# braingeneers/statdepth

Hardware: AMD Instinct MI355X
Metric: curve-pairs/sec (MBD) (higher is better)
Workload: dtype f64

## Files before the change

statdepth_amd/csrc/mbd_rank_bucket32.hip:

```cpp
#include <atomic>

#include "sd_common.h"
#include "rank_routes.h"
#include "rank_bucket.h"

namespace sd {

constexpr int R32_PRIO_LDS = 2;
constexpr int R32_PRIO_VALU = 0;
constexpr int R32_MIN_N = 3072;
constexpr int R32_LNB = 14;
constexpr int R32_NT = 512, R32_NW = 8;
constexpr int R32_LCAP = 64;
constexpr int R32_PAD = 12;
constexpr u32 R32_TB = 1024;
constexpr int R32_TSH = 30;
constexpr double R32_CDIV = 1.0 / 448.0;
constexpr double R32_BETA = 2.0;
constexpr double R32_VBASE = 274877906944.0;
constexpr u32 R32_VBASE_HI = 0x42500000u;
constexpr u32 R32_SENT = 0x7FFFFFFFu;

__device__ __forceinline__ u32 r32_word_offset(u32 vh) { return (vh << 2) & 0xFFFCu; }
__device__ __forceinline__ u32 r32_key_word(u32 off4, u32 par) { return (off4 << 5) | (par << 3); }
__device__ __forceinline__ u32 r32_key_word_offset(u32 kw) { return __builtin_amdgcn_ubfe(kw, 5u, 16u); }
__device__ __forceinline__ u32 r32_key_word_bucket(u32 kw) { return (__builtin_amdgcn_ubfe(kw, 7u, 14u) << 1) | ((kw >> 3) & 1u); }
__device__ __forceinline__ u32 r32_pair_word(u32 base, u32 h) { return __builtin_amdgcn_perm(base, h, 0x05040200u); }
__device__ __forceinline__ void r32_pair_decode(u32 pw, u32 kw, u32 &base, u32 &cnt) {
    cnt = __builtin_amdgcn_ubfe(pw, kw, 8u);
    base = (pw >> 16) + __builtin_amdgcn_ubfe(pw, 0u, kw);
}

template <int E, int LNB>
struct R32Cfg {
    static constexpr int NT = R32_NT, NW = R32_NW, NB = 1 << LNB;
    static constexpr int QW = NB / 2 / NT / 4;
    static_assert(QW >= 1 && NB / 2 == QW * 4 * NT, "whole quads of histogram words per thread");
    static constexpr int SH = 31 - LNB;
    static constexpr u32 C0 = R32_TB << SH, C1 = ((u32)NB - R32_TB) << SH;
    static constexpr u32 CU0 = 2u << SH, CU1 = ((u32)NB - 2u) << SH;
    static_assert(C0 % (2u << SH) == 0 && C1 % (2u << SH) == 0 && CU0 % (2u << SH) == 0 && CU1 % (2u << SH) == 0,
                  "the core's bounds are whole steps of the high word of 2^38 + image (2^18 images)");
    static constexpr u32 NANIMG = ((u32)NB + 2u) << SH;
    static_assert(LNB == 14, "the first tail octave continues the core's slope for 14 336 core buckets");
    static constexpr size_t HDR = 8 * NW * 8 + NW * 4 + 32 + (size_t)R32_LCAP * 8;
    static_assert(HDR % 16 == 0, "the histogram starts on a 16-byte boundary");
    static __host__ __device__ constexpr int al4(int n) { return (n + 3) & ~3; }
    static __host__ __device__ constexpr int pstride(int n) { return (n + 31) & ~31; }
    static __host__ __device__ constexpr int dummy_pos(int n) { return al4(n) + R32_PAD; }
    static __host__ __device__ constexpr size_t lds_bytes(int n) { return HDR + (size_t)(NB / 2 + 4) * 4 + (size_t)(dummy_pos(n) + 4) * 4; }
};

template <int E, int LNB>
__global__ __launch_bounds__(R32_NT, 4) void rank_bucket32_kernel(const double *__restrict__ Y, i64 n64, i64 row0, i64 rows,
                                                                 u32 *__restrict__ partial, unsigned char *__restrict__ rowflag,
                                                                 u32 *__restrict__ gate, u32 epoch, u64 *__restrict__ out_zero) {
    using C = R32Cfg<E, LNB>;
    constexpr int NT = C::NT, NW = C::NW, NB = C::NB, QW = C::QW, SH = C::SH;
    constexpr u32 C0 = C::C0, C1 = C::C1, CU0 = C::CU0, CU1 = C::CU1, NANIMG = C::NANIMG;
    constexpr size_t LDS = C::lds_bytes(E * NT);
    static_assert(2 * LDS <= 160 * 1024, "two workgroups per CU");
    static_assert(R32_PAD >= 0 && C::al4(E * NT) + 3 < C::dummy_pos(E * NT) + 4, "the second quad of the last bucket lies in S");
    __shared__ __attribute__((aligned(16))) double Sm[(LDS + 7) / 8];
    const int n = (int)n64;
    double *red = Sm;
    u32 *wtot = reinterpret_cast<u32 *>(red + 8 * NW);
    u32 *misc = wtot + NW;
    u32 *lkey = misc + 8, *lbe = lkey + R32_LCAP;
    u32 *H = reinterpret_cast<u32 *>(reinterpret_cast<char *>(Sm) + C::HDR);
    u32 *S = H + NB / 2 + 4;
    const unsigned short *H16 = reinterpret_cast<const unsigned short *>(H);
    const int t0 = threadIdx.x;
    const double INF = __builtin_huge_val();
    const double QNAN = __builtin_nan("");
    const int DUMMY = C::dummy_pos(n);
    const u32 nm1 = (u32)n - 1u;
    const u32 ranksum = (u32)(((u64)n * (u64)(n - 1)) >> 1);
    int t = t0;

    if (blockIdx.x == 0 && t == 0) gate[2] = 0;
    if (out_zero)
        for (i64 c = (i64)blockIdx.x * NT + t; c < n; c += (i64)gridDim.x * NT) out_zero[c] = 0;
    for (int p = n + t; p < DUMMY + 4; p += NT) S[p] = R32_SENT;
    {
        uint4 *Hq = reinterpret_cast<uint4 *>(H);
#pragma unroll
        for (int i = 0; i < QW; ++i) Hq[i * NT + t] = make_uint4(0, 0, 0, 0);
        if (t < 4) H[NB / 2 + t] = 0;
        if (t < 5) misc[t] = 0;
    }

    double x[E];
    auto load_row = [&](i64 r) {
        const double *rp = Y + (row0 + r) * n + t;
#pragma unroll
        for (int e = 0; e < E; ++e) x[e] = (e < E - 2 || t + e * NT < n) ? rp[e * NT] : QNAN;
    };
    u32 acc[E];
#pragma unroll
    for (int e = 0; e < E; ++e) acc[e] = 0;
    auto row_range = [&](int parity) {
        double mn = INF, mx = -INF;
#pragma unroll
        for (int e = 0; e < E; ++e) {
            mn = rb_mm<false>(mn, x[e]);
            mx = rb_mm<true>(mx, x[e]);
        }
        float2 wb = rb3_wave_bracket<E, NT>(mn, mx);
        {
            bool eqs = false;
#pragma unroll
            for (int e = 0; e < (E - 1 < 10 ? E - 1 : 10); ++e) eqs = eqs || (x[e] == x[e + 1]);
            if (__ballot(eqs) != 0) {
                float finf = __builtin_huge_valf();
                asm volatile("" : "+v"(finf));
                wb.x = finf;
                wb.y = -finf;
            }
        }
        const float imn = wb.x, imx = wb.y;
        mn = rb_wave_allreduce<false>(mn);
        mx = rb_wave_allreduce<true>(mx);
        double *rp = red + parity * 4 * NW;
        if ((t & 63) == 63) {
            double *wp = rp + 4 * (t >> 6);
            wp[0] = mn; wp[1] = mx;
            reinterpret_cast<float *>(wp + 2)[0] = imn;
            reinterpret_cast<float *>(wp + 2)[1] = imx;
        }
    };
    int par = 0;
    u32 rowidx = 0, nbad = 0, expect = 0;
    bool handover = false;
    bool stop = false;
    u32 kb[E];
    i64 r = blockIdx.x;
    for (; r < rows; r += gridDim.x) {
        t = t0;
        asm volatile("" : "+v"(t));
        const int lane = t & 63;
        const int wave = __builtin_amdgcn_readfirstlane(t >> 6);
        if (rowidx && t == 0) misc[3] = __hip_atomic_load(gate + 1, __ATOMIC_RELAXED, __HIP_MEMORY_SCOPE_AGENT);
        __builtin_amdgcn_s_setprio(R32_PRIO_LDS);
        load_row(r);
        row_range(par);
        double *redp = red + par * 4 * NW;
        par ^= 1;
        __syncthreads();
        if (rowidx) {
            const u32 w = misc[3];
            if ((w >> 8) == (epoch & 0xFFFFFFu) && (w & 0xFFu) >= 8u) { stop = true; break; }
        }
        double lo, hi;
        double mscale, moff, mc;
        u64 mcb;
        u32 mc0, mcw;
        u32 mh0, mhw;
        bool go, bad;
        {
            const double2 p = reinterpret_cast<const double2 *>(redp)[2 * (lane & (NW - 1))];
            const float2 pb = reinterpret_cast<const float2 *>(redp + 4 * (lane & (NW - 1)) + 2)[0];
            lo = rb_readlane_f64(rb_row_allreduce<false>(p.x), 0);
            hi = rb_readlane_f64(rb_row_allreduce<true>(p.y), 0);
            const double imn = (double)__int_as_float(__builtin_amdgcn_readfirstlane(__float_as_int(rb_row_allreduce_f32<true>(pb.x))));
            const double imx = (double)__int_as_float(__builtin_amdgcn_readfirstlane(__float_as_int(rb_row_allreduce_f32<false>(pb.y))));
            const bool fin = (hi > lo) && (lo > -INF) && (hi < INF) && ((hi - lo) < INF);
            bad = !fin && (hi >= lo);
            const double si = imx - imn;
            u32 c0 = CU0, c1 = CU1;
            if (fin && si > 0.0 && si < INF && (hi - lo) > (1.5 * (1.0 + 2.0 * R32_BETA)) * si) {
                const double lo2 = imn - R32_BETA * si, hi2 = imx + R32_BETA * si;
                lo = lo2 > lo ? lo2 : lo;
                hi = hi2 < hi ? hi2 : hi;
                c0 = C0;
                c1 = C1;
            }
            mc0 = c0;
            mcw = c1 - c0;
            const double wc = hi - lo;
            mscale = ((double)mcw - 64.0) / wc;
            moff = __builtin_fma(-lo, mscale, R32_VBASE + (double)c0);
            mh0 = R32_VBASE_HI + (c0 >> (SH + 1));
            mhw = mcw >> (SH + 1);
            mc = wc * R32_CDIV;
            mcb = (u64)__double_as_longlong(mc);
            go = fin && (wc > 0.0) && (mscale < INF) && (mc > 0.0);
            bad = bad || (fin && !go);
        }
        auto convert4 = [&](const double (&xv)[4], const bool (&isk)[4], u32 (&q)[4], u32 (&bk)[4]) {
            bool anyout = false;
            u32 vh[4];
#pragma unroll
            for (int i = 0; i < 4; ++i) {
                const u64 w = (u64)__double_as_longlong(__builtin_fma(xv[i], mscale, moff));
                vh[i] = (u32)(w >> 32);
                q[i] = (u32)w;
                anyout = anyout || (isk[i] && vh[i] - mh0 >= mhw);
            }
            if (__ballot(anyout) != 0) {
                const double vlo = __longlong_as_double((long long)((u64)mh0 << 32));
                double zero = 0.0;
                asm volatile("" : "+v"(zero));
#pragma unroll
                for (int i = 0; i < 4; ++i) {
                    const bool outc = vh[i] - mh0 >= mhw;
                    const bool low = __longlong_as_double((long long)(((u64)vh[i] << 32) | q[i])) < vlo;
                    double d = low ? lo - xv[i] : xv[i] - hi;
                    d = rb_mm<true>(d, zero);
                    const u64 tc = ((u64)__double_as_longlong(d + mc) - mcb) >> R32_TSH;
                    const u32 room = low ? mc0 - 1u : 0x7FFFFEFFu - (mc0 + mcw);
                    const u32 tcc = tc < (u64)room ? (u32)tc : room;
                    u32 qt = low ? (mc0 - 1u) - tcc : (mc0 + mcw) + tcc;
                    qt = (xv[i] == xv[i]) ? qt : NANIMG;
                    vh[i] = outc ? qt >> (SH + 1) : vh[i];
                    q[i] = outc ? qt << (31 - SH) : q[i];
                }
            }
#pragma unroll
            for (int i = 0; i < 4; ++i) {
                vh[i] = isk[i] ? vh[i] : NANIMG >> (SH + 1);
                q[i] = isk[i] ? q[i] : NANIMG << (31 - SH);
                bk[i] = vh[i];
            }
        };
        u32 bc[E];
        if (go) {

#pragma unroll
            for (int e0 = 0; e0 < E; e0 += 8) {
                u32 old[8];
#pragma unroll
                for (int h = 0; h < 8; h += 4) {
                    if (e0 + h < E) {
                        double xv[4];
                        u32 q[4], bk[4];
                        bool isk[4];
#pragma unroll
                        for (int i = 0; i < 4; ++i) {
                            const int e = e0 + h + i < E ? e0 + h + i : e0 + h;
                            xv[i] = x[e];
                            isk[i] = e < E - 2 || t + e * NT < n;
                        }
                        convert4(xv, isk, q, bk);
#pragma unroll
                        for (int i = 0; i < 4; ++i)
                            if (e0 + h + i < E) { kb[e0 + h + i] = q[i]; bc[e0 + h + i] = bk[i]; }
                    }
                }
#pragma unroll
                for (int i = 0; i < 8; ++i) {
                    const int e = e0 + i;
                    if (e < E) {
                        const u32 off4 = r32_word_offset(bc[e]);
                        u32 par = kb[e] >> 31, one;
                        asm("v_mad_u32_u24 %0, %1, %2, 1" : "=v"(one) : "v"(par), "s"(0xFFFFu));
                        asm("" : "+v"(par));
                        old[i] = atomicAdd(reinterpret_cast<u32 *>(reinterpret_cast<char *>(H) + off4), one);
                        bc[e] = r32_key_word(off4, par);
                    }
                }
#pragma unroll
                for (int i = 0; i < 8; ++i) {
                    const int e = e0 + i;
                    if (e < E)
                        bc[e] |= __builtin_amdgcn_ubfe(old[i], bc[e] << 1, 8u) << 24;
                }
#pragma unroll
                for (int i = 0; i < 8; ++i)
                    if (e0 + i < E) asm volatile("" : "+v"(bc[e0 + i]));
            }
            __syncthreads();
            uint4 *Hq = reinterpret_cast<uint4 *>(H) + wave * (64 * QW);
            uint4 hq[QW];
            u32 runq[QW], inclq[QW], offq[QW], ov = 0, wsum = 0;
#pragma unroll
            for (int i = 0; i < QW; ++i) {
                hq[i] = Hq[i * 64 + lane];
                const u32 s4 = hq[i].x + hq[i].y + hq[i].z + hq[i].w;
                ov |= hq[i].x | hq[i].y | hq[i].z | hq[i].w;
                runq[i] = (s4 & 0xFFFFu) + (s4 >> 16);
                inclq[i] = rb_wave_incl_scan(runq[i]);
                offq[i] = wsum;
                wsum += rb_readlane(inclq[i], 63);
            }
            const bool wover = __ballot((ov & 0xFFC0FFC0u) != 0) != 0;
            const bool wtry = __ballot((ov & 0xFFF0FFF0u) != 0) != 0;
            if (lane == 63) wtot[wave] = wsum | (wover ? 0x80000000u : 0u) | (wtry ? 0x40000000u : 0u);
            __syncthreads();
            const u32 wt = wtot[lane & (NW - 1)];
            const bool crowded = __ballot((wt >> 31) != 0) != 0;
            const bool trypure = __ballot((wt & 0x40000000u) != 0) != 0;
            const u32 wscan = rb_row_incl_scan(wt & 0x3FFFFFFFu);
            const u32 woff = wave ? rb_readlane(wscan, wave - 1) : 0u;
#pragma unroll
            for (int i = 0; i < QW; ++i) {
                const u32 b0 = woff + offq[i] + inclq[i] - runq[i];
                const u32 b1 = b0 + (hq[i].x & 0xFFFFu) + (hq[i].x >> 16);
                const u32 b2 = b1 + (hq[i].y & 0xFFFFu) + (hq[i].y >> 16);
                const u32 b3 = b2 + (hq[i].z & 0xFFFFu) + (hq[i].z >> 16);
                uint4 o;
                if (!crowded) {
                    o.x = r32_pair_word(b0, hq[i].x);
                    o.y = r32_pair_word(b1, hq[i].y);
                    o.z = r32_pair_word(b2, hq[i].z);
                    o.w = r32_pair_word(b3, hq[i].w);
                } else {
                    o.x = b0 | ((b0 + (hq[i].x & 0xFFFFu)) << 16);
                    o.y = b1 | ((b1 + (hq[i].y & 0xFFFFu)) << 16);
                    o.z = b2 | ((b2 + (hq[i].z & 0xFFFFu)) << 16);
                    o.w = b3 | ((b3 + (hq[i].w & 0xFFFFu)) << 16);
                }
                Hq[i * 64 + lane] = o;
                if (i == QW - 1 && t == NT - 1)
                    H[NB / 2] = b3 + (hq[i].w & 0xFFFFu) + (hq[i].w >> 16);
            }
            __syncthreads();
            const u32 nv = H[NB / 2];
            bool take = nv == (u32)n;
            if (take && !crowded) {
#pragma unroll
                for (int e = 0; e < E; ++e) {
                    const u32 pw = *reinterpret_cast<const u32 *>(reinterpret_cast<const char *>(H) + r32_key_word_offset(bc[e]));
                    __builtin_amdgcn_sched_barrier(0);
                    u32 base, cnt;
                    r32_pair_decode(pw, bc[e], base, cnt);
                    const bool isk = e < E - 2 || t + e * NT < n;
                    *reinterpret_cast<u32 *>(reinterpret_cast<char *>(S) + (isk ? (base << 2) + (bc[e] >> 22) : (u32)DUMMY * 4u)) = kb[e];
                    bc[e] = isk ? base | (cnt << 14) : (1u << 14);
                }
            } else if (take) {
#pragma unroll
                for (int e = 0; e < E; ++e) {
                    const u32 b = r32_key_word_bucket(bc[e]), slot = bc[e] >> 24;
                    u32 b1 = b + 1u;
                    asm("" : "+v"(b1));
                    const u32 base = H16[b], end = H16[b1];
                    const bool isk = e < E - 2 || t + e * NT < n;
                    S[isk ? base + slot : (u32)DUMMY] = kb[e];
                    bc[e] = isk ? base | ((end - base) << 14) : (1u << 14);
                }
            }
            __syncthreads();
            bool pure = false;
            if (take && (trypure || crowded)) {
                const u32 tag = rowidx + 1u;
                bool vote = false, same = true;
#pragma unroll
                for (int e = 0; e < E; ++e) {
                    const u32 base = bc[e] & 0x3FFFu, cnt = bc[e] >> 14;
                    if (e < E - 2 || t + e * NT < n) {
                        const u32 first = S[base];
                        same = same && (first == kb[e]);
                        if (cnt >= 16u) vote = vote || (first == kb[e] && S[base + 1] == kb[e]);
                    }
                }
                if (vote) misc[2] = tag;
                if (!same) misc[4] = tag;
                __syncthreads();
                if ((misc[2] == tag && misc[4] != tag) || crowded) {
                    take = false;
                    bool ok = misc[2] == tag && misc[4] != tag;
                    if (ok) {
                        const double *rp = Y + (row0 + r) * n + t;
#pragma unroll
                        for (int pass = 0; pass < 2; ++pass) {
                            bool eq = true;
#pragma unroll
                            for (int e0 = 0; e0 < E; e0 += 4) {
                                int eo = e0 * NT;
                                asm volatile("" : "+v"(eo));
                                const double *rq = rp + eo;
                                u64 w[4];
#pragma unroll
                                for (int i = 0; i < 4; ++i) {
                                    const bool isk = e0 + i < E && (e0 + i < E - 2 || t + (e0 + i) * NT < n);
                                    w[i] = (u64)__double_as_longlong((isk ? rq[i * NT] : 0.0) + 0.0);
                                }
#pragma unroll
                                for (int i = 0; i < 4; ++i) {
                                    if (e0 + i < E && (e0 + i < E - 2 || t + (e0 + i) * NT < n) && (bc[e0 + i] >> 14) >= 2u) {
                                        u32 *sp = S + (bc[e0 + i] & 0x3FFFu);
                                        if (pass == 0) { sp[0] = (u32)(w[i] >> 32); sp[1] = (u32)w[i]; }
                                        else eq = eq && sp[0] == (u32)(w[i] >> 32) && sp[1] == (u32)w[i];
                                    }
                                }
                                __builtin_amdgcn_sched_barrier(0);
                            }
                            if (pass == 1 && !eq) misc[4] = tag;
                            __syncthreads();
                        }
                        ok = misc[4] != tag;
                    }
                    if (ok) {
                        pure = true;
#pragma unroll
                        for (int e = 0; e < E; ++e) {
                            const u32 B = bc[e] & 0x3FFFu, A = (u32)n - B - (bc[e] >> 14);
                            acc[e] += (e < E - 2 || t + e * NT < n) ? (nm1 * (nm1 - 1u) - A * (A - 1u) - B * (B - 1u)) >> 1 : 0u;
                        }
                    }
                }
            }
            __builtin_amdgcn_s_setprio(R32_PRIO_VALU);
            {
                uint4 *Hz = reinterpret_cast<uint4 *>(H) + wave * (64 * QW);
#pragma unroll
                for (int i = 0; i < QW; ++i) Hz[i * 64 + lane] = make_uint4(0, 0, 0, 0);
                if (t < 2) H[NB / 2 + t] = 0;
            }
            if (take) {
                const uint4 *S4 = reinterpret_cast<const uint4 *>(S);
                uint4 y0, y1;
                auto window = [&](int e) {
                    const u32 base = bc[e] & 0x3FFFu;
                    const uint4 *p = S4 + (base >> 2);
                    y0 = p[0];
                    y1 = p[1];
                };
                u32 sB = 0;
                window(0);
#pragma unroll
                for (int e = 0; e < E; ++e) {
                    const u32 base = bc[e] & 0x3FFFu, cnt = bc[e] >> 14, off = base & 3u;
                    const u32 qe = kb[e];
                    u32 lt = 0;
                    lt = __builtin_amdgcn_alignbit(lt, y1.w - qe, 31);
                    lt = __builtin_amdgcn_alignbit(lt, y1.z - qe, 31);
                    lt = __builtin_amdgcn_alignbit(lt, y1.y - qe, 31);
                    lt = __builtin_amdgcn_alignbit(lt, y1.x - qe, 31);
                    lt = __builtin_amdgcn_alignbit(lt, y0.w - qe, 31);
                    lt = __builtin_amdgcn_alignbit(lt, y0.z - qe, 31);
                    lt = __builtin_amdgcn_alignbit(lt, y0.y - qe, 31);
                    lt = __builtin_amdgcn_alignbit(lt, y0.x - qe, 31);
                    if (e + 1 < E) window(e + 1);
                    u32 less = (u32)__popc(__builtin_amdgcn_ubfe(lt, off, cnt < 8u ? cnt : 8u));
                    if (cnt + off > 8u) {
                        const uint4 *p = S4 + (base >> 2);
#pragma unroll 1
                        for (u32 kk = 8; kk < cnt + off; kk += 4) {
                            const uint4 y = p[kk >> 2];
                            const u32 rest = cnt + off - kk;
                            u32 l4 = 0;
                            l4 = __builtin_amdgcn_alignbit(l4, y.w - qe, 31);
                            l4 = __builtin_amdgcn_alignbit(l4, y.z - qe, 31);
                            l4 = __builtin_amdgcn_alignbit(l4, y.y - qe, 31);
                            l4 = __builtin_amdgcn_alignbit(l4, y.x - qe, 31);
                            less += (u32)__popc(__builtin_amdgcn_ubfe(l4, 0u, rest < 4u ? rest : 4u));
                        }
                    }
                    const u32 B = base + less;
                    kb[e] = B;
                    const bool isk = e < E - 2 || t + e * NT < n;
                    sB += isk ? B : 0u;
                    acc[e] += isk ? __umul24(B, nm1 - B) : 0u;
                    __builtin_amdgcn_sched_barrier(0);
                }
                sB = rb_wave_incl_scan(sB);
                if (lane == 63) atomicAdd(&misc[1], sB);
                __syncthreads();
                {
                    const u32 have_sum = misc[1];
                    expect += ranksum;
                    if (have_sum != expect) {
                        expect = have_sum;
                        const u32 l0 = misc[0];
#pragma unroll
                        for (int e = 0; e < E; ++e)
                            if (e < E - 2 || t + e * NT < n) atomicAdd(&H[kb[e] >> 1], 1u << ((kb[e] & 1u) * 16u));
                        __syncthreads();
#pragma unroll
                        for (int e = 0; e < E; ++e) {
                            if (e < E - 2 || t + e * NT < n) {
                                const u32 B = kb[e], c = H16[B];
                                if (c != 1u) {
                                    acc[e] -= __umul24(B, nm1 - B);
                                    const u32 idx = atomicAdd(&misc[0], 1u);
                                    if (idx < (u32)R32_LCAP) {
                                        lkey[idx] = (rowidx << 14) | (u32)(t + e * NT);
                                        lbe[idx] = B | (c << 16);
                                    }
                                }
                            }
                        }
                        __syncthreads();
                        if (E <= 16 && misc[0] > (u32)R32_LCAP) {
                            const u32 tag = (rowidx + 1u) | 0x40000000u;
                            const double *rp = Y + (row0 + r) * n + t;
#pragma unroll
                            for (int pass = 0; pass < 2; ++pass) {
                                bool eq = true;
#pragma unroll
                                for (int e0 = 0; e0 < E; e0 += 2) {
                                    int eo = e0 * NT;
                                    asm volatile("" : "+v"(eo));
                                    const double *rq = rp + eo;
                                    u64 w[2];
#pragma unroll
                                    for (int i = 0; i < 2; ++i) {
                                        const bool isk = e0 + i < E && (e0 + i < E - 2 || t + (e0 + i) * NT < n);
                                        w[i] = (u64)__double_as_longlong((isk ? rq[i * NT] : 0.0) + 0.0);
                                    }
#pragma unroll
                                    for (int i = 0; i < 2; ++i) {
                                        if (e0 + i < E && (e0 + i < E - 2 || t + (e0 + i) * NT < n) && H16[kb[e0 + i]] >= 2u) {
                                            u32 *sp = S + kb[e0 + i];
                                            if (pass == 0) { sp[0] = (u32)(w[i] >> 32); sp[1] = (u32)w[i]; }
                                            else eq = eq && sp[0] == (u32)(w[i] >> 32) && sp[1] == (u32)w[i];
                                        }
                                    }
                                    __builtin_amdgcn_sched_barrier(0);
                                }
                                if (pass == 1 && !eq) misc[4] = tag;
                                __syncthreads();
                            }
                            if (misc[4] != tag) {
#pragma unroll
                                for (int e = 0; e < E; ++e) {
                                    if (e < E - 2 || t + e * NT < n) {
                                        const u32 B = kb[e], c = H16[B];
                                        if (c != 1u) {
                                            const u32 A = (u32)n - B - c;
                                            acc[e] += (nm1 * (nm1 - 1u) - A * (A - 1u) - B * (B - 1u)) >> 1;
                                        }
                                    }
                                }
                                if (t == 0) misc[0] = l0;
                            }
                            __syncthreads();
                        }
#pragma unroll
                        for (int e = 0; e < E; ++e)
                            if (e < E - 2 || t + e * NT < n) H[kb[e] >> 1] = 0;
                        __syncthreads();
                        if (misc[0] > (u32)R32_LCAP) handover = true;
                    }
                }
            } else {
                bad = !pure;
            }
        }
        if (t == 0) rowflag[r] = bad ? 1 : 0;
        nbad += bad ? 1u : 0u;
        ++rowidx;
        if (handover) break;
        if (bad && rowidx == 1 && t == 0 && blockIdx.x < 16) {
            u32 old = gate[1], assumed;
            do {
                assumed = old;
                const u32 want = ((assumed >> 8) != (epoch & 0xFFFFFFu)) ? (((epoch & 0xFFFFFFu) << 8) | 1u)
                                 : ((assumed & 0xFFu) == 0xFFu ? assumed : assumed + 1u);
                old = atomicCAS(gate + 1, assumed, want);
            } while (old != assumed);
        }
        if (nbad >= 2 && 2 * nbad > rowidx) { stop = true; r += gridDim.x; break; }
    }
    t = t0;
    __syncthreads();
    const u32 L = __builtin_amdgcn_readfirstlane(handover ? 0u : misc[0]);
    if (handover) {
        for (i64 rr = blockIdx.x + (i64)t * gridDim.x; rr < rows; rr += (i64)NT * gridDim.x) rowflag[rr] = 1;
        nbad = 1;
#pragma unroll
        for (int e = 0; e < E; ++e) acc[e] = 0;
    } else if (stop) {
        for (i64 rr = r + (i64)t * gridDim.x; rr < rows; rr += (i64)NT * gridDim.x) rowflag[rr] = 1;
    }
    if (t == 0 && nbad) *gate = epoch;
    u32 key = 0, be = 0;
    double xv = 0.0;
    if ((u32)t < L) {
        key = lkey[t];
        be = lbe[t];
        xv = Y[(row0 + (i64)blockIdx.x + (i64)(key >> 14) * gridDim.x) * n + (key & 0x3FFFu)];
    }
    u32 *P = partial + (size_t)blockIdx.x * C::pstride(n);
#pragma unroll
    for (int e = 0; e < E; ++e)
        if (e < E - 2 || t + e * NT < n) __builtin_nontemporal_store(acc[e], &P[t + e * NT]);
    if (L) {
        asm volatile("s_waitcnt vmcnt(0)" ::: "memory");
        __syncthreads();
        if (t < 64) {
            u32 B = be & 0xFFFFu, A = (u32)n - B - (be >> 16);
            for (u32 j = 0; j < L; ++j) {
                const u32 kj = rb_readlane(key, (int)j), bj = rb_readlane(be, (int)j);
                const double xj = rb_readlane_f64(xv, (int)j);
                if (j != (u32)t && (kj >> 14) == (key >> 14) && (bj & 0xFFFFu) == (be & 0xFFFFu)) {
                    B += (xj < xv) ? 1u : 0u;
                    A += (xj > xv) ? 1u : 0u;
                }
            }
            if ((u32)t < L) atomicAdd(&P[key & 0x3FFFu], (nm1 * (nm1 - 1u) - A * (A - 1u) - B * (B - 1u)) >> 1);
        }
    }
}

bool rank_bucket32_supported(i64 n, i64 rows, int cus) {
    const u64 per = (u64)((rows + cus - 1) / cus) * (u64)n * (u64)n;
    return n > R32_MIN_N && n <= 11264 && rows >= cus && rows <= 4096 && per < ((u64)1 << 32) && xswitch("SD_RB_NO32") == 0;
}

size_t rank_bucket32_extra_bytes(i64 rows) { return align_up((size_t)rows + 64, 256); }

template <int E>
static int launch32_cfg(const double *Y, i64 n, i64 row0, i64 rows, u32 *partial, unsigned char *rowflag, u32 *gate, u32 epoch,
                        u64 *out_zero, int G, hipStream_t s) {
    auto kf = rank_bucket32_kernel<E, R32_LNB>;
    if (n > (i64)E * R32_NT || n <= (i64)(E - 2) * R32_NT)
        return fail(SD_ERR_UNSUPPORTED, "bucket32 kernel: n=%lld is not of the class E=%d", (long long)n, E);
    hipLaunchKernelGGL(kf, dim3(G), dim3(R32_NT), 0, s, Y, n, row0, rows, partial, rowflag, gate, epoch, out_zero);
    SD_HIP(hipGetLastError());
    return SD_OK;
}

int launch_rank_bucket32(const double *Y, i64 n, i64 row0, i64 rows, u32 *partial, unsigned char *rowflag, u32 *gate, u32 epoch,
                         u64 *out_zero, int G, hipStream_t s) {
    switch ((int)((n + 1023) / 1024)) {
        case 3: return launch32_cfg<6>(Y, n, row0, rows, partial, rowflag, gate, epoch, out_zero, G, s);
        case 4: return launch32_cfg<8>(Y, n, row0, rows, partial, rowflag, gate, epoch, out_zero, G, s);
        case 5: return launch32_cfg<10>(Y, n, row0, rows, partial, rowflag, gate, epoch, out_zero, G, s);
        case 6: return launch32_cfg<12>(Y, n, row0, rows, partial, rowflag, gate, epoch, out_zero, G, s);
        case 7: return launch32_cfg<14>(Y, n, row0, rows, partial, rowflag, gate, epoch, out_zero, G, s);
        case 8: return launch32_cfg<16>(Y, n, row0, rows, partial, rowflag, gate, epoch, out_zero, G, s);
        case 9: return launch32_cfg<18>(Y, n, row0, rows, partial, rowflag, gate, epoch, out_zero, G, s);
        case 10: return launch32_cfg<20>(Y, n, row0, rows, partial, rowflag, gate, epoch, out_zero, G, s);
        case 11: return launch32_cfg<22>(Y, n, row0, rows, partial, rowflag, gate, epoch, out_zero, G, s);
    }
    return fail(SD_ERR_UNSUPPORTED, "bucket32 kernel covers 3072 < n <= 11264");
}

u32 rank_bucket32_epoch() {
    static std::atomic<u32> counter{0};
    u32 e = ++counter;
    if (e == 0) e = ++counter;
    return e;
}

}
```

Baseline: 2544 billion.

## Prefetch next row's data into registers during current row's rank pass

Moves the global load of the next row's values out of the loop head and issues it in two halves during the current row's processing: the low half after the histogram clear and the high half midway through the rank loop, or on the fallback paths. The aim is to hide global memory latency behind the LDS-heavy rank computation. In exchange, the x registers now hold the next row while the current row is still in flight, which raises register pressure. Several asm volatile barriers are added to keep the kb values from being rematerialised and to steer scheduling.

```diff
diff --git a/statdepth_amd/csrc/mbd_rank_bucket32.hip b/statdepth_amd/csrc/mbd_rank_bucket32.hip
--- a/statdepth_amd/csrc/mbd_rank_bucket32.hip
+++ b/statdepth_amd/csrc/mbd_rank_bucket32.hip
@@ -1,4 +1,5 @@
 #include <atomic>
+#include <type_traits>
 
 #include "sd_common.h"
 #include "rank_routes.h"
@@ -91,16 +92,23 @@
     }
 
     double x[E];
-    auto load_row = [&](i64 r) {
-        const double *rp = Y + (row0 + r) * n + t;
-#pragma unroll
-        for (int e = 0; e < E; ++e) x[e] = (e < E - 2 || t + e * NT < n) ? rp[e * NT] : QNAN;
+    auto load_row = [&](i64 r, auto half, bool real) {
+        constexpr int E0 = half.value == 2 ? E / 2 : 0, E1 = half.value == 1 ? E / 2 : E;
+        const double *rp = Y + (row0 + r) * n;
+        const u32 tu = real ? (u32)t : 0u;
+#pragma unroll
+        for (int e = E0; e < E1; ++e) x[e] = (e < E - 2 || t + e * NT < n) ? (rp + e * NT)[tu] : QNAN;
     };
+    using RowAll = std::integral_constant<int, 0>;
+    using RowLo = std::integral_constant<int, 1>;
+    using RowHi = std::integral_constant<int, 2>;
     u32 acc[E];
 #pragma unroll
     for (int e = 0; e < E; ++e) acc[e] = 0;
     auto row_range = [&](int parity) {
-        double mn = INF, mx = -INF;
+        u32 zw, pw, nw;
+        asm volatile("v_mov_b32 %0, 0\n\tv_mov_b32 %1, 0x7ff00000\n\tv_mov_b32 %2, 0xfff00000" : "=v"(zw), "=v"(pw), "=v"(nw));
+        double mn = __hiloint2double((int)pw, (int)zw), mx = __hiloint2double((int)nw, (int)zw);
 #pragma unroll
         for (int e = 0; e < E; ++e) {
             mn = rb_mm<false>(mn, x[e]);
@@ -133,8 +141,8 @@
     u32 rowidx = 0, nbad = 0, expect = 0;
     bool handover = false;
     bool stop = false;
-    u32 kb[E];
     i64 r = blockIdx.x;
+    load_row(r < rows ? r : rows - 1, RowAll{}, true);
     for (; r < rows; r += gridDim.x) {
         t = t0;
         asm volatile("" : "+v"(t));
@@ -142,7 +150,6 @@
         const int wave = __builtin_amdgcn_readfirstlane(t >> 6);
         if (rowidx && t == 0) misc[3] = __hip_atomic_load(gate + 1, __ATOMIC_RELAXED, __HIP_MEMORY_SCOPE_AGENT);
         __builtin_amdgcn_s_setprio(R32_PRIO_LDS);
-        load_row(r);
         row_range(par);
         double *redp = red + par * 4 * NW;
         par ^= 1;
@@ -223,7 +230,10 @@
                 bk[i] = vh[i];
             }
         };
+        u32 kb[E];
         u32 bc[E];
+        const bool have = r + gridDim.x < rows;
+        const i64 rnext = have ? r + gridDim.x : r;
         if (go) {
 
 #pragma unroll
@@ -408,6 +418,7 @@
                 for (int i = 0; i < QW; ++i) Hz[i * 64 + lane] = make_uint4(0, 0, 0, 0);
                 if (t < 2) H[NB / 2 + t] = 0;
             }
+            load_row(rnext, RowLo{}, have);
             if (take) {
                 const uint4 *S4 = reinterpret_cast<const uint4 *>(S);
                 uint4 y0, y1;
@@ -448,12 +459,17 @@
                             less += (u32)__popc(__builtin_amdgcn_ubfe(l4, 0u, rest < 4u ? rest : 4u));
                         }
                     }
-                    const u32 B = base + less;
+                    u32 B = base + less;
+                    asm volatile("" : "+v"(B));
                     kb[e] = B;
                     const bool isk = e < E - 2 || t + e * NT < n;
                     sB += isk ? B : 0u;
                     acc[e] += isk ? __umul24(B, nm1 - B) : 0u;
                     __builtin_amdgcn_sched_barrier(0);
+                    if (e == E / 2 - 1) {
+                        load_row(rnext, RowHi{}, have);
+                        __builtin_amdgcn_sched_barrier(0);
+                    }
                 }
                 sB = rb_wave_incl_scan(sB);
                 if (lane == 63) atomicAdd(&misc[1], sB);
@@ -465,13 +481,18 @@
                         expect = have_sum;
                         const u32 l0 = misc[0];
 #pragma unroll
-                        for (int e = 0; e < E; ++e)
-                            if (e < E - 2 || t + e * NT < n) atomicAdd(&H[kb[e] >> 1], 1u << ((kb[e] & 1u) * 16u));
+                        for (int e = 0; e < E; ++e) {
+                            u32 k = kb[e];
+                            asm volatile("" : "+v"(k));
+                            if (e < E - 2 || t + e * NT < n) atomicAdd(&H[k >> 1], 1u << ((k & 1u) * 16u));
+                        }
                         __syncthreads();
 #pragma unroll
                         for (int e = 0; e < E; ++e) {
                             if (e < E - 2 || t + e * NT < n) {
-                                const u32 B = kb[e], c = H16[B];
+                                u32 B = kb[e];
+                                asm volatile("" : "+v"(B));
+                                const u32 c = H16[B];
                                 if (c != 1u) {
                                     acc[e] -= __umul24(B, nm1 - B);
                                     const u32 idx = atomicAdd(&misc[0], 1u);
@@ -529,15 +550,22 @@
                             __syncthreads();
                         }
 #pragma unroll
-                        for (int e = 0; e < E; ++e)
-                            if (e < E - 2 || t + e * NT < n) H[kb[e] >> 1] = 0;
+                        for (int e = 0; e < E; ++e) {
+                            u32 k = kb[e];
+                            asm volatile("" : "+v"(k));
+                            if (e < E - 2 || t + e * NT < n) H[k >> 1] = 0;
+                        }
                         __syncthreads();
                         if (misc[0] > (u32)R32_LCAP) handover = true;
                     }
                 }
             } else {
                 bad = !pure;
-            }
+                load_row(rnext, RowHi{}, have);
+                __builtin_amdgcn_s_waitcnt(0x0F70);
+            }
+        } else {
+            load_row(rnext, RowAll{}, have);
         }
         if (t == 0) rowflag[r] = bad ? 1 : 0;
         nbad += bad ? 1u : 0u;
```

Result: faster. 2588 billion (median of 6 runs) (+1.7%).
